# polimi-ispl/deep_prior_interpolation

Hardware: AMD Instinct MI355X
Metric: Adam iters/sec on 3D MultiRes-UNet (whole job over n_gpus; per_gpu beside it); recon SNR(dB) vs ref under config.snr_vs_reference (higher is better)
Workload: dtype f32

## Files before the change

### deep_prior_interpolation_amd/csrc/api.cpp

```cpp
#include <stdarg.h>
#include <string.h>
#include "common.h"

static thread_local char g_err[512] = "";

void dpi_set_error(const char* fmt, ...) {
  va_list ap;
  va_start(ap, fmt);
  vsnprintf(g_err, sizeof(g_err), fmt, ap);
  va_end(ap);
}

int dpi_check_launch(const char* what) {
  const hipError_t e = hipGetLastError();
  if (e != hipSuccess) {
    dpi_set_error("%s: %s", what, hipGetErrorString(e));
    return DPI_E_LAUNCH;
  }
  return DPI_OK;
}

extern "C" const char* dpi_last_error(void) { return g_err; }
extern "C" int dpi_version(void) { return 406; }
extern "C" int dpi_conv_desc_size(void) { return (int)sizeof(dpi_conv_desc); }

extern "C" int dpi_device_info(int device, int* cus, int* lds_bytes, size_t* hbm_bytes, char* name, int name_len) {
  hipDeviceProp_t p;
  const hipError_t e = hipGetDeviceProperties(&p, device);
  if (e != hipSuccess) {
    dpi_set_error("device_info: %s", hipGetErrorString(e));
    return DPI_E_LAUNCH;
  }
  if (cus) *cus = p.multiProcessorCount;
  if (lds_bytes) *lds_bytes = (int)p.sharedMemPerBlock;
  if (hbm_bytes) *hbm_bytes = p.totalGlobalMem;
  if (name && name_len > 0) {
    strncpy(name, p.gcnArchName, name_len - 1);
    name[name_len - 1] = 0;
  }
  return DPI_OK;
}

__global__ void dpi_marker_kernel() {}

extern "C" int dpi_profile_marker(int id, void* stream) {
  DPI_REQUIRE(id >= 1 && id < 65536, "profile_marker: id %d out of range", id);
  dpi_marker_kernel<<<(unsigned)id, 64, 0, (hipStream_t)stream>>>();
  return dpi_check_launch("profile_marker");
}

extern "C" int dpi_set_option(const char* key, int value) {
  DPI_REQUIRE(key != nullptr, "set_option: key is NULL");
  struct Entry { const char* key; int lo, hi; void (*set)(int); };
  static const Entry table[] = {
      {"splitk", 0, 1, dpi_set_splitk},
      {"dual_bwd_data", 0, 1, dpi_set_dual_bwd_data},
      {"bw_pair", 0, 2, dpi_set_bw_pair},
      {"bw_workgroups", 1, 1 << 24, [](int v) { dpi_set_bw_tuning(v, -1); }},
      {"bw_xcd_order", 0, 1, [](int v) { dpi_set_bw_tuning(0, v); }},
      {"mfma_min_cout", 0, 1 << 20, dpi_set_mfma_min_cout},
      {"bwd_weight_mfma_min_cout", 0, 1 << 20, dpi_set_bwd_weight_mfma_min_cout},
      {"fewco_mfma", 0, 1, dpi_set_fewco_mfma},
      {"q4", 0, 2, [](int v) { dpi_set_q4(v, -1); }},
      {"q4_ck", 0, 4, [](int v) { dpi_set_q4(-1, v); }},
      {"q4_debug", 0, 0xFFFF, dpi_set_q4_debug},
      {"bf16_debug", 0, 0x7F, dpi_set_bf16_debug},
  };
  for (const Entry& e : table)
    if (strcmp(key, e.key) == 0) {
      DPI_REQUIRE(value >= e.lo && value <= e.hi && !(strcmp(key, "q4_ck") == 0 && value != 0 && value != 2 && value != 4),
                  "set_option: %s = %d out of range [%d, %d]", key, value, e.lo, e.hi);
      e.set(value);
      return DPI_OK;
    }
  dpi_set_error("set_option: unknown key '%s'", key);
  return DPI_E_ARG;
}
```

### deep_prior_interpolation_amd/csrc/conv_mfma.hip

```cpp
#include "common.h"

void dpi_conv_out_dims(const dpi_conv_desc* d, int* Do, int* Ho, int* Wo);

namespace {

typedef float f32x4 __attribute__((ext_vector_type(4)));

struct MArgs {
  const float* __restrict__ x;
  const float* __restrict__ chain;
  const float* __restrict__ w;
  const float* __restrict__ bias;
  float* __restrict__ y;
  double* __restrict__ partials;
  int Cin, Cout;
  int D, H, W;
  int ntd, nth, ntw;
  long w_out_stride, w_in_stride;
  int accumulate;
  int split_cps;
  const float* __restrict__ x2;
  const float* __restrict__ w2;
  int C2;
  long w2_co_stride, w2_c_stride;
  int xb, yb;
  int ny;
};

template <int KD, int NR, int NH, int S = 1>
struct Geo {
  static constexpr bool SLICES = (KD == 3 && NR >= 4);
  static constexpr int SD = KD == 3 ? S : 1;
  static constexpr int TZ = SLICES ? 4 : 1;
  static constexpr int TY = SLICES ? NR : 4 * NR;
  static constexpr int TW = 16 * NH;
  static constexpr int ID = (TZ - 1) * SD + KD;
  static constexpr int IH = (TY - 1) * S + 3;
  static constexpr int IW = (TW - 1) * S + 3;
  static constexpr int RS = (IW + 3) & ~3;
  static constexpr int DS0 = IH * RS;
  static constexpr int DS = (S == 1 && (RS % 32) == 4) ? DS0 + ((12 - (DS0 % 32)) + 32) % 32 : DS0;
  static constexpr int CS0 = ID * DS;
  static constexpr int CSM = S == 1 ? 16 : 1;
  static constexpr int CS = CS0 + ((CSM - (CS0 % 32)) + 32) % 32;
  static constexpr int TILE = ID * IH * IW;
  static constexpr int E = (TILE + 255) / 256;
  static constexpr int NROW = (NR - 1) * S + 3;
  static constexpr int NSTEP = KD * NROW;
  static constexpr int NB = 3 * NH;
};

__device__ __forceinline__ int xcd_tile(int bid, int ntiles) {
  const int q = ntiles >> 3, r = ntiles & 7, xcd = bid & 7, i = bid >> 3;
  return (xcd < r ? xcd * (q + 1) : r * (q + 1) + (xcd - r) * q) + i;
}

template <class G>
__device__ __forceinline__ void tile_slots(int tid, int id0, int ih0, int iw0, int D, int H, int W, int (&goff)[G::E], int (&loff)[G::E]) {
#pragma unroll
  for (int e = 0; e < G::E; ++e) {
    const int idx = tid + e * 256;
    const int col = idx % G::IW, row = idx / G::IW;
    const int hy = row % G::IH, dz = row / G::IH;
    const int gd = id0 + dz, gh = ih0 + hy, gw = iw0 + col;
    const bool ok = idx < G::TILE && gd >= 0 && gd < D && gh >= 0 && gh < H && gw >= 0 && gw < W;
    goff[e] = ok ? (gd * H + gh) * W + gw : -1;
    loff[e] = idx < G::TILE ? dz * G::DS + hy * G::RS + col : -1;
  }
}

template <class G>
__device__ __forceinline__ void stage_load(float (&sr)[4][G::E], const float* __restrict__ x, int Cin, size_t V, int c0,
                                           const int (&goff)[G::E], bool xb = false) {
  if (xb) {
#pragma unroll
    for (int c = 0; c < 4; ++c) {
      const int ci = min(c0 + c, Cin - 1);
      const __amdgpu_buffer_rsrc_t r = dpi_buffer_t(dpi_at(x, (size_t)ci * V, true), V, true);
#pragma unroll
      for (int e = 0; e < G::E; ++e) sr[c][e] = dpi_buffer_load_bf16_raw(r, goff[e]);
    }
    return;
  }
#pragma unroll
  for (int c = 0; c < 4; ++c) {
    const int ci = min(c0 + c, Cin - 1);
    const __amdgpu_buffer_rsrc_t r = dpi_buffer(x + (size_t)ci * V, V * sizeof(float));
#pragma unroll
    for (int e = 0; e < G::E; ++e) sr[c][e] = dpi_buffer_load(r, goff[e] * 4);
  }
}

template <class G>
__device__ __forceinline__ void stage_store(float* lds, const float (&sr_in)[4][G::E], const float* __restrict__ chain, int Cin, int c0,
                                            const int (&goff)[G::E], const int (&loff)[G::E], bool xb = false) {
  float sr[4][G::E];
#pragma unroll
  for (int c = 0; c < 4; ++c)
#pragma unroll
    for (int e = 0; e < G::E; ++e) sr[c][e] = sr_in[c][e];
  if (xb) {
#pragma unroll
    for (int c = 0; c < 4; ++c)
#pragma unroll
      for (int e = 0; e < G::E; ++e) sr[c][e] = dpi_widen_raw(sr[c][e]);
  }
  if (chain == nullptr) {
#pragma unroll
    for (int c = 0; c < 4; ++c)
#pragma unroll
      for (int e = 0; e < G::E; ++e)
        if ((e + 1) * 256 <= G::TILE || loff[e] >= 0) lds[c * G::CS + loff[e]] = sr[c][e];
    return;
  }
#pragma unroll
  for (int c = 0; c < 4; ++c) {
    const int ci = min(c0 + c, Cin - 1);
    const Chain t = load_chain(chain, ci);
#pragma unroll
    for (int e = 0; e < G::E; ++e) {
      const float v = goff[e] >= 0 ? apply_chain(t, sr[c][e]) : sr[c][e];
      if ((e + 1) * 256 <= G::TILE || loff[e] >= 0) lds[c * G::CS + loff[e]] = v;
    }
  }
}

template <int KD, int NR, int NH>
struct GeoV2 {
  static constexpr int TY = 4 * NR, TW = 16 * NH;
  static constexpr int ID = KD == 3 ? 3 : 1, IH = (TY - 1) * 2 + 3;
  static constexpr int NQ = TW / 2 + 1;
  static constexpr int PW = 2 * NQ;
  static constexpr int RS = 2 * PW;
  static constexpr int DS = IH * RS;
  static constexpr int CS0 = ID * DS;
  static constexpr int CS = CS0 + ((16 - (CS0 % 32)) + 32) % 32;
  static constexpr int NV4 = ID * IH * NQ;
  static constexpr int E = (NV4 + 255) / 256;
};
template <class GV>
__device__ __forceinline__ void tile_slots_v(int tid, int id0, int ih0, int iw0, int D, int H, int W, int (&goff)[GV::E], int (&loff)[GV::E]) {
#pragma unroll
  for (int e = 0; e < GV::E; ++e) {
    const int idx = tid + e * 256;
    const int q = idx % GV::NQ, row = idx / GV::NQ;
    const int hy = row % GV::IH, dz = row / GV::IH;
    const int gd = id0 + dz, gh = ih0 + hy, gw = iw0 + 4 * q;
    const bool ok = idx < GV::NV4 && gd >= 0 && gd < D && gh >= 0 && gh < H && gw >= 0 && gw + 4 <= W;
    goff[e] = ok ? (gd * H + gh) * W + gw : -4;
    loff[e] = idx < GV::NV4 ? dz * GV::DS + hy * GV::RS + 2 * q : -1;
  }
}
template <class GV>
// ... 877 lines not shown
      for (int t = 0; t < TAPS; ++t) wr[t] = ok ? wn[t] : 0.f;
    }
    __syncthreads();
#pragma unroll
    for (int c = 0; c < 4; ++c)
#pragma unroll
      for (int e = 0; e < E; ++e)
        if ((e + 1) * 256 <= TILE || loff[e] >= 0) lds[c * CS + loff[e]] = a.dyb ? dpi_widen_raw(sr[c][e]) : sr[c][e];
    __syncthreads();
    if (c0 + 4 < a.Cout) fetch(c0 + 4);
#pragma unroll
    for (int sd = 0; sd < ID; ++sd)
#pragma unroll
      for (int ir = 0; ir < 3; ++ir)
#pragma unroll
        for (int sw = 0; sw < 2; ++sw) {
          const float b = lds[lbase + (sd * IH + ir) * RS + sw];
#pragma unroll
          for (int sh = 0; sh < 2; ++sh) {
            const int row = ir - sh;
            if (row < 0 || row > 1) continue;
#pragma unroll
            for (int cls = 0; cls < NCLS; ++cls) {
              const int pw = cls & 1, ph = (cls >> 1) & 1, pd = KD == 3 ? (cls >> 2) & 1 : 0;
              if ((sw && !pw) || (sh && !ph) || (sd && !pd)) continue;
              const int kw = pw ? (sw ? 0 : 2) : 1, kh = ph ? (sh ? 0 : 2) : 1, kd = KD == 3 ? (pd ? (sd ? 0 : 2) : 1) : 0;
              acc[cls][row] = __builtin_amdgcn_mfma_f32_16x16x4f32(wr[(kd * 3 + kh) * 3 + kw], b, acc[cls][row], 0, 0, 0);
            }
          }
        }
  }
  typedef float f32x2 __attribute__((ext_vector_type(2)));
  const bool vec2 = !a.dxb && ((a.W | (int)(V & 1)) & 1) == 0 && (((uintptr_t)a.dx) & 7) == 0;
  if (vec2) {
#pragma unroll
    for (int cp = 0; cp < NCLS / 2; ++cp) {
      const int ph = cp & 1, pd = KD == 3 ? (cp >> 1) & 1 : 0;
#pragma unroll
      for (int row = 0; row < 2; ++row) {
        const int id = KD == 3 ? 2 * md0 + pd : md0, ih = 2 * (mh0 + wid * 2 + row) + ph, iw = 2 * (mw0 + lj);
        if (id < a.D && ih < a.H && iw < a.W) {
          f32x2 old[4];
#pragma unroll
          for (int r = 0; r < 4; ++r) {
            const int ci = n0 + 4 * lk + r;
            const size_t o = (size_t)min(ci, a.Cin - 1) * V + ((size_t)id * a.H + ih) * a.W + iw;
            old[r] = a.accumulate ? *reinterpret_cast<const f32x2*>(a.dx + o) : (f32x2){0.f, 0.f};
          }
#pragma unroll
          for (int r = 0; r < 4; ++r) {
            const int ci = n0 + 4 * lk + r;
            if (ci < a.Cin) {
              const size_t o = (size_t)ci * V + ((size_t)id * a.H + ih) * a.W + iw;
              const f32x2 v = a.accumulate ? (f32x2){old[r][0] + acc[2 * cp][row][r], old[r][1] + acc[2 * cp + 1][row][r]}
                                           : (f32x2){acc[2 * cp][row][r], acc[2 * cp + 1][row][r]};
              *reinterpret_cast<f32x2*>(a.dx + o) = v;
            }
          }
        }
      }
    }
    return;
  }
#pragma unroll
  for (int cls = 0; cls < NCLS; ++cls) {
    const int pw = cls & 1, ph = (cls >> 1) & 1, pd = KD == 3 ? (cls >> 2) & 1 : 0;
#pragma unroll
    for (int row = 0; row < 2; ++row) {
      const int id = KD == 3 ? 2 * md0 + pd : md0, ih = 2 * (mh0 + wid * 2 + row) + ph, iw = 2 * (mw0 + lj) + pw;
      if (id < a.D && ih < a.H && iw < a.W) {
#pragma unroll
        for (int r = 0; r < 4; ++r) {
          const int ci = n0 + 4 * lk + r;
          if (ci < a.Cin) {
            const size_t o = (size_t)ci * V + ((size_t)id * a.H + ih) * a.W + iw;
            dpi_st(a.dx, o, a.accumulate ? dpi_ld(a.dx, o, a.dxb) + acc[cls][row][r] : acc[cls][row][r], a.dxb);
          }
        }
      }
    }
  }
}

__global__ __launch_bounds__(256) void splitk_reduce_kernel(const float* __restrict__ ws, int nsplit, const float* __restrict__ bias,
                                                            float* __restrict__ y, int accumulate, double* __restrict__ partials,
                                                            int Cout, size_t Vo, size_t per, bool yb) {
  const int lane = threadIdx.x & 63, co = blockIdx.y * 4 + (threadIdx.x >> 6);
  if (co >= Cout) return;
  const size_t lo = (size_t)blockIdx.x * per, hi = lo + per < Vo ? lo + per : Vo;
  const float bv = bias ? bias[co] : 0.f;
  double sum = 0.0, sq = 0.0;
  for (size_t v = lo + lane; v < hi; v += 64) {
    float t = ws[(size_t)co * Vo + v];
    for (int sp = 1; sp < nsplit; ++sp) t += ws[((size_t)sp * Cout + co) * Vo + v];
    t += bv;
    if (accumulate) t += dpi_ld(y, (size_t)co * Vo + v, yb);
    t = dpi_stored(t, yb);
    dpi_st(y, (size_t)co * Vo + v, t, yb);
    sum += t; sq += (double)t * t;
  }
  if (partials) {
#pragma unroll
    for (int o = 32; o > 0; o >>= 1) { sum += __shfl_xor(sum, o, 64); sq += __shfl_xor(sq, o, 64); }
    if (lane == 0) { partials[((size_t)blockIdx.x * Cout + co) * 2] = sum; partials[((size_t)blockIdx.x * Cout + co) * 2 + 1] = sq; }
  }
}

}

void dpi_mfma_variant(const dpi_conv_desc* d, int cout, int* nr, int* nh) {
  int Do, Ho, Wo;
  dpi_conv_out_dims(d, &Do, &Ho, &Wo);
  const int tz = d->kd == 3 ? 4 : 1, ty = d->kd == 3 ? 8 : 32;
  const long nb = (long)cdiv(Do, tz) * cdiv(Ho, ty) * cdiv(Wo, 32) * cdiv(cout, 16);
  if (nb >= 512 && d->stride == 1) { *nr = 8; *nh = 2; }
  else { *nr = 2; *nh = Wo > 16 ? 2 : 1; }
}

bool dpi_mfma_half_tile(const dpi_conv_desc* d, bool flip) {
  const int cin = flip ? d->Cout : d->Cin, cout = flip ? d->Cin : d->Cout;
  int nr, nh;
  dpi_mfma_variant(d, cout, &nr, &nh);
  if (nr != 8 || d->kd != 3) return false;
  if (cin == 1) return true;
  if (cin <= 8) return false;
  return flip || ((cin & 3) == 1);
}

int dpi_mfma_tiles(const dpi_conv_desc* d, int nr, int nh, int* ntd, int* nth, int* ntw) {
  int Do, Ho, Wo;
  dpi_conv_out_dims(d, &Do, &Ho, &Wo);
  const bool slices = d->kd == 3 && nr >= 4;
  const int tz = slices ? 4 : 1, ty = slices ? nr : 4 * nr;
  *ntd = cdiv(Do, tz); *nth = cdiv(Ho, ty); *ntw = cdiv(Wo, 16 * nh);
  return *ntd * *nth * *ntw;
}

template <int KD, bool FLIP, bool IOB = false>
static void launch_variant(const MArgs& a_in, int nr, int nh, int stride, dim3 grid_in, hipStream_t st) {
  if constexpr (!IOB) {
    if (a_in.xb || a_in.yb) { launch_variant<KD, FLIP, true>(a_in, nr, nh, stride, grid_in, st); return; }
  }
  const bool persistent = stride == 1 && nr == 8 && a_in.Cin > 8;
  MArgs a = a_in;
  dim3 grid = grid_in;
  if (!persistent && grid_in.y > 1) {
    a.ny = (int)grid_in.y;
    grid = dim3(8 * ((grid_in.x + 7) / 8) * grid_in.y, 1, grid_in.z);
  }
  if (stride == 2) {
    if constexpr (!FLIP) {
      if constexpr (!IOB) {
        static const bool s2v = getenv("DPI_NO_S2V") == nullptr;
        if (s2v && a.W % 4 == 0 && (((size_t)a.D * a.H * a.W) & 3) == 0 && ((uintptr_t)a.x & 15) == 0) {
          if (nh == 2) conv_mfma_kernel<KD, 2, 2, false, 2, 2, false, false, false, false, true><<<grid, 256, 0, st>>>(a);
          else conv_mfma_kernel<KD, 2, 1, false, 2, 2, false, false, false, false, true><<<grid, 256, 0, st>>>(a);
          return;
        }
      }
      if (nh == 2) conv_mfma_kernel<KD, 2, 2, false, 2, 2, false, false, IOB><<<grid, 256, 0, st>>>(a);
      else conv_mfma_kernel<KD, 2, 1, false, 2, 2, false, false, IOB><<<grid, 256, 0, st>>>(a);
    }
    return;
  }
  const bool tailpack = (a.Cin & 3) == 1 && (a.Cin > 4 || a.Cin == 1);
  if (nr == 4) {
    if constexpr (KD == 3) {
      if (tailpack) conv_mfma_kernel<KD, 4, 2, FLIP, 1, 3, false, true, IOB><<<grid, 256, 0, st>>>(a);
      else conv_mfma_kernel<KD, 4, 2, FLIP, 1, 3, false, false, IOB><<<grid, 256, 0, st>>>(a);
    }
    return;
  }
  if (nr == 8) {
    static const bool persist = getenv("DPI_NO_PERSIST") == nullptr;
    dim3 pg = grid;
    static const bool yloop = getenv("DPI_YLOOP") != nullptr && getenv("DPI_YLOOP")[0] == '1';
    if constexpr (KD == 3 && FLIP && !IOB) {
      if (yloop && a.Cin <= 4 && a.ny > 1 && a.split_cps == 0 && grid_in.z == 1) {
        conv_mfma_kernel<KD, 8, 2, FLIP, 1, 2, false, false, IOB, true><<<dim3(8 * ((grid_in.x + 7) / 8), 1, 1), 256, 0, st>>>(a);
        return;
      }
    }
    if (a.Cin <= 8) conv_mfma_kernel<KD, 8, 2, FLIP, 1, 3, false, false, IOB><<<grid, 256, 0, st>>>(a);
    else {
      if (persist && grid.x > 512) pg.x = 512;
      if (tailpack) conv_mfma_kernel<KD, 8, 2, FLIP, 1, 2, true, true, IOB><<<pg, 256, 0, st>>>(a);
      else conv_mfma_kernel<KD, 8, 2, FLIP, 1, 2, true, false, IOB><<<pg, 256, 0, st>>>(a);
    }
  }
  else if (nh == 2) conv_mfma_kernel<KD, 2, 2, FLIP, 1, 2, false, false, IOB><<<grid, 256, 0, st>>>(a);
  else conv_mfma_kernel<KD, 2, 1, FLIP, 1, 2, false, false, IOB><<<grid, 256, 0, st>>>(a);
}

#ifdef DPI_TRACE
extern "C" int dpi_debug_read_blocks(long long* out) { return (int)hipMemcpyFromSymbol(out, HIP_SYMBOL(g_blk), sizeof(long long) * 8192 * 4); }
extern "C" int dpi_debug_read_trace(long long* out) { return (int)hipMemcpyFromSymbol(out, HIP_SYMBOL(g_trace), sizeof(long long) * 4 * 64); }
#endif
static int g_splitk = getenv("DPI_SPLITK") ? atoi(getenv("DPI_SPLITK")) : 1;
extern "C" void dpi_set_splitk(int on) { g_splitk = on; }
int dpi_mfma_splitk(const dpi_conv_desc* d, bool flip) {
  if (!g_splitk || d->k != 3) return 1;
  const int cin = flip ? d->Cout : d->Cin, cout = flip ? d->Cin : d->Cout;
  int nr, nh, a, b, c;
  dpi_mfma_variant(d, cout, &nr, &nh);
  if (nr != 2 || dpi_mfma_half_tile(d, flip)) return 1;
  const long wgs = (long)dpi_mfma_tiles(d, nr, nh, &a, &b, &c) * cdiv(cout, 16);
  const int chunks = cdiv(cin, 4);
  if (wgs > 512 || (wgs > 256 && chunks < 24)) return 1;
  long ns = 1536 / wgs;
  if (ns > chunks / 8) ns = chunks / 8;
  if (ns > 8) ns = 8;
  return ns < 2 ? 1 : (int)ns;
}
size_t dpi_conv_mfma_ws_floats(const dpi_conv_desc* d, bool flip) {
  const int ns = dpi_mfma_splitk(d, flip);
  if (ns < 2) return 0;
  int Do, Ho, Wo;
  dpi_conv_out_dims(d, &Do, &Ho, &Wo);
  return (size_t)ns * (flip ? d->Cin : d->Cout) * Do * Ho * Wo;
}

bool dpi_conv_mfma_second_ok(const dpi_conv_desc* d, bool flip, int C2, bool have_ws) {
  int Do, Ho, Wo;
  dpi_conv_out_dims(d, &Do, &Ho, &Wo);
  if (!flip || d->stride != 1 || C2 < 1 || ((size_t)C2 + 4) * Do * Ho * Wo * sizeof(float) >= ((size_t)1 << 31)) return false;
  int nr, nh;
  dpi_mfma_variant(d, d->Cin, &nr, &nh);
  if (nr == 8 && !dpi_mfma_half_tile(d, flip) && d->Cout > 8) return false;
  return !(have_ws && dpi_mfma_splitk(d, flip) > 1);
}

int dpi_conv_mfma_run(const dpi_conv_desc* d, const float* x, const float* chain, const float* w, const float* bias, float* y,
                      double* partials, bool flip, int accumulate, float* ws, size_t ws_floats, hipStream_t st, const MfmaSecond* sec) {
  const int taps = d->kd * 9;
  const int cin = flip ? d->Cout : d->Cin, cout = flip ? d->Cin : d->Cout;
  const long w_out = flip ? taps : (long)d->Cin * taps, w_in = flip ? (long)d->Cin * taps : taps;
  MArgs a{x, chain, w, bias, y, partials, cin, cout, d->D, d->H, d->W, 0, 0, 0, w_out, w_in, accumulate, 0, nullptr, nullptr, 0, 0, 0,
          dpi_io_in(d, flip), dpi_io_out(d, flip)};
  int nr, nh;
  dpi_mfma_variant(d, cout, &nr, &nh);
  if (dpi_mfma_half_tile(d, flip)) nr = 4;
  const int ntiles = dpi_mfma_tiles(d, nr, nh, &a.ntd, &a.nth, &a.ntw);
  dim3 grid(ntiles, cdiv(cout, 16));
  if (sec) { a.x2 = sec->x2; a.w2 = sec->w2; a.C2 = sec->C2; a.w2_co_stride = sec->w2_co_stride; a.w2_c_stride = sec->w2_c_stride; }
  const int nsplit = (ws && !sec) ? dpi_mfma_splitk(d, flip) : 1;
  if (nsplit > 1) {
    int Do, Ho, Wo;
    dpi_conv_out_dims(d, &Do, &Ho, &Wo);
    const size_t Vo = (size_t)Do * Ho * Wo;
    DPI_REQUIRE(ws_floats >= (size_t)nsplit * cout * Vo, "conv (split): workspace of %zu floats, need %zu", ws_floats, (size_t)nsplit * cout * Vo);
    a.split_cps = 4 * cdiv(cdiv(cin, 4), nsplit);
    a.y = ws; a.bias = nullptr; a.partials = nullptr; a.accumulate = 0; a.yb = 0;
    grid.z = cdiv(cin, a.split_cps);
    const int nz = (int)grid.z;
    if (d->kd == 3) { if (flip) launch_variant<3, true>(a, nr, nh, d->stride, grid, st); else launch_variant<3, false>(a, nr, nh, d->stride, grid, st); }
    else { if (flip) launch_variant<1, true>(a, nr, nh, d->stride, grid, st); else launch_variant<1, false>(a, nr, nh, d->stride, grid, st); }
    if (int e = dpi_check_launch("conv_mfma (split)")) return e;
    splitk_reduce_kernel<<<dim3(ntiles, cdiv(cout, 4)), 256, 0, st>>>(ws, nz, bias, y, accumulate, partials, cout, Vo, cdivz(Vo, (size_t)ntiles),
                                                                      dpi_io_out(d, flip));
    return dpi_check_launch("splitk_reduce");
  }
  if (d->kd == 3) { if (flip) launch_variant<3, true>(a, nr, nh, d->stride, grid, st); else launch_variant<3, false>(a, nr, nh, d->stride, grid, st); }
  else { if (flip) launch_variant<1, true>(a, nr, nh, d->stride, grid, st); else launch_variant<1, false>(a, nr, nh, d->stride, grid, st); }
  return dpi_check_launch("conv_mfma");
}

static bool mfma_bw_swap_better(const dpi_conv_desc* d) {
  if (d->stride != 1) return false;
  auto util = [](int rows, int staged) { return (double)rows / (16.0 * cdiv(rows, 16)) * staged / (4.0 * cdiv(staged, 4)); };
  return util(d->Cin, d->Cout) > 1.15 * util(d->Cout, d->Cin);
}

static int g_bw_want = getenv("DPI_BW_WANT") ? atoi(getenv("DPI_BW_WANT")) : 2304;
static int g_bw_xcd_order = getenv("DPI_BW_XCD_ORDER") ? atoi(getenv("DPI_BW_XCD_ORDER")) : 0;
extern "C" void dpi_set_bw_tuning(int want_workgroups, int xcd_order) {
  if (want_workgroups > 0) g_bw_want = want_workgroups;
  if (xcd_order >= 0) g_bw_xcd_order = xcd_order;
}
static size_t bw_extra_lds() { static const size_t v = getenv("DPI_BW_EXTRA_LDS") ? (size_t)atoi(getenv("DPI_BW_EXTRA_LDS")) * 1024 : 0; return v; }
struct MfmaBwPlan { int nchunks, tiles_per_chunk, ntiles, ntd, nth, ntw, nr, nh, npairs, nfull, ny; };
static int g_bw_pair = getenv("DPI_BW_PAIR") ? atoi(getenv("DPI_BW_PAIR")) : 2;
extern "C" void dpi_set_bw_pair(int mode) { if (mode >= 0 && mode <= 2) g_bw_pair = mode; }
static MfmaBwPlan mfma_bw_plan(const dpi_conv_desc* d, bool swap = false) {
  MfmaBwPlan p{};
  {
    const int staged = swap ? d->Cout : d->Cin, groups = cdiv(staged, 4);
    const bool s1k3 = d->stride == 1 && d->kd == 3;
    const int tailg = (s1k3 && (staged & 3) == 1) ? 1 : 0;
    p.nfull = groups - tailg;
    p.npairs = (g_bw_pair && s1k3 && !g_bw_xcd_order && p.nfull >= 2 && d->io == 0) ? p.nfull / 2 : 0;
    if (g_bw_pair == 2) {
      int a_, b_, c_;
      if (p.nfull < 4 || dpi_mfma_tiles(d, 8, 2, &a_, &b_, &c_) < 1024) p.npairs = 0;
    }
    p.ny = p.npairs ? p.npairs + (p.nfull & 1) + tailg : groups;
  }
  if (d->stride == 1) { p.nr = 8; p.nh = 2; }
  else { int Do, Ho, Wo; dpi_conv_out_dims(d, &Do, &Ho, &Wo); p.nr = 2; p.nh = Wo > 16 ? 2 : 1; }
  p.ntiles = dpi_mfma_tiles(d, p.nr, p.nh, &p.ntd, &p.nth, &p.ntw);
  const size_t per = (size_t)d->Cout * d->Cin * d->kd * 9;
  const size_t max_chunks_mem = per ? ((size_t)32 << 20) / per : 1;
  const size_t blocks_other = (size_t)p.ny * (swap ? cdiv(d->Cin, 16) : cdiv(d->Cout, 16));
  size_t want = (size_t)g_bw_want / blocks_other;
  if (want < 1) want = 1;
  if (want > (size_t)p.ntiles) want = p.ntiles;
  if (want > max_chunks_mem) want = max_chunks_mem;
// ... 134 lines not shown
```

### deep_prior_interpolation_amd/csrc/dpi_hip_internal.h

```cpp
#pragma once
#define DPI_INTERNAL __attribute__((visibility("hidden")))
extern "C" {
DPI_INTERNAL void dpi_set_bw_tuning(int want_workgroups, int xcd_order);
DPI_INTERNAL void dpi_set_bf16_debug(int flags);
DPI_INTERNAL void dpi_set_splitk(int on);
DPI_INTERNAL void dpi_set_dual_bwd_data(int on);
DPI_INTERNAL void dpi_set_bw_pair(int mode);
DPI_INTERNAL void dpi_set_mfma_min_cout(int n);
DPI_INTERNAL void dpi_set_bwd_weight_mfma_min_cout(int n);
DPI_INTERNAL void dpi_set_fewco_mfma(int on);
DPI_INTERNAL void dpi_set_q4(int on, int ck);
DPI_INTERNAL void dpi_set_q4_debug(int flags);
}
```

Before: 33.97.

## Add dedicated stride-2 forward MFMA conv kernel with multi-Cout-tile register reuse

Adds a new stride-2 3x3x3 forward conv kernel that deinterleaves even and odd input columns into LDS, keeps all 27 weight taps in registers, and computes two 16-wide output-channel groups per block (MT=2). This reuses each staged input tile across more output channels and prefetches the next channel chunk's input and weights while the current one computes. It is enabled by default when the layer has at least two Cout groups. The cost is higher register pressure and a new code path that duplicates the epilogue and stats-partials logic.

```diff
diff --git a/deep_prior_interpolation_amd/csrc/api.cpp b/deep_prior_interpolation_amd/csrc/api.cpp
--- a/deep_prior_interpolation_amd/csrc/api.cpp
+++ b/deep_prior_interpolation_amd/csrc/api.cpp
@@ -65,6 +65,7 @@
       {"q4_ck", 0, 4, [](int v) { dpi_set_q4(-1, v); }},
       {"q4_debug", 0, 0xFFFF, dpi_set_q4_debug},
       {"bf16_debug", 0, 0x7F, dpi_set_bf16_debug},
+      {"s2_fwd", 0, 2, dpi_set_s2_fwd},
   };
   for (const Entry& e : table)
     if (strcmp(key, e.key) == 0) {
diff --git a/deep_prior_interpolation_amd/csrc/conv_mfma.hip b/deep_prior_interpolation_amd/csrc/conv_mfma.hip
--- a/deep_prior_interpolation_amd/csrc/conv_mfma.hip
+++ b/deep_prior_interpolation_amd/csrc/conv_mfma.hip
@@ -1,4 +1,5 @@
 #include "common.h"
+#include "conv_s2_mfma.h"
 
 void dpi_conv_out_dims(const dpi_conv_desc* d, int* Do, int* Ho, int* Wo);
 
@@ -1182,6 +1183,14 @@
     if constexpr (!FLIP) {
       if constexpr (!IOB) {
         static const bool s2v = getenv("DPI_NO_S2V") == nullptr;
+        if constexpr (KD == 3) {
+          const S2FwdArgs f{a.x, a.chain, a.w, a.bias, a.y, a.partials, a.Cin, a.Cout, a.D, a.H, a.W, a.ntd, a.nth, a.ntw,
+                            a.w_out_stride, a.w_in_stride, a.accumulate, a.split_cps, (int)grid_in.y};
+          if (a.x2 == nullptr && dpi_conv_s2_fwd_wanted(f)) {
+            dpi_conv_s2_fwd_launch(f, nh, (int)grid_in.x, (int)grid_in.z, st);
+            return;
+          }
+        }
         if (s2v && a.W % 4 == 0 && (((size_t)a.D * a.H * a.W) & 3) == 0 && ((uintptr_t)a.x & 15) == 0) {
           if (nh == 2) conv_mfma_kernel<KD, 2, 2, false, 2, 2, false, false, false, false, true><<<grid, 256, 0, st>>>(a);
           else conv_mfma_kernel<KD, 2, 1, false, 2, 2, false, false, false, false, true><<<grid, 256, 0, st>>>(a);
diff --git a/deep_prior_interpolation_amd/csrc/conv_s2_mfma.h b/deep_prior_interpolation_amd/csrc/conv_s2_mfma.h
--- /dev/null
+++ b/deep_prior_interpolation_amd/csrc/conv_s2_mfma.h
@@ -0,0 +1,23 @@
+#pragma once
+#include <hip/hip_runtime.h>
+
+struct S2FwdArgs {
+  const float* x;
+  const float* chain;
+  const float* w;
+  const float* bias;
+  float* y;
+  double* partials;
+  int Cin, Cout;
+  int D, H, W;
+  int ntd, nth, ntw;
+  long w_out_stride, w_in_stride;
+  int accumulate;
+  int split_cps;
+  int ny;
+};
+
+int dpi_s2_fwd_mode();
+bool dpi_conv_s2_fwd_can(const S2FwdArgs& a);
+bool dpi_conv_s2_fwd_wanted(const S2FwdArgs& a);
+void dpi_conv_s2_fwd_launch(const S2FwdArgs& a, int nh, int ntiles, int nz, hipStream_t st);
diff --git a/deep_prior_interpolation_amd/csrc/conv_s2_mfma.hip b/deep_prior_interpolation_amd/csrc/conv_s2_mfma.hip
--- /dev/null
+++ b/deep_prior_interpolation_amd/csrc/conv_s2_mfma.hip
@@ -0,0 +1,287 @@
+#include <stdlib.h>
+#include "common.h"
+#include "conv_s2_mfma.h"
+
+namespace {
+
+typedef float f32x4 __attribute__((ext_vector_type(4)));
+typedef float f32x2 __attribute__((ext_vector_type(2)));
+
+template <int NH>
+struct S2Geo {
+  static constexpr int NR = 2, TY = 4 * NR, TW = 16 * NH;
+  static constexpr int ID = 3, IH = (TY - 1) * 2 + 3;
+  static constexpr int NQ = TW / 2 + 1;
+  static constexpr int PW = 2 * NQ;
+  static constexpr int RS = 2 * PW;
+  static constexpr int DS = IH * RS;
+  static constexpr int CS0 = ID * DS;
+  static constexpr int CS = CS0 + ((16 - (CS0 % 32)) + 32) % 32;
+  static constexpr int NV4 = ID * IH * NQ;
+  static constexpr int E = (NV4 + 255) / 256;
+  static constexpr int NROW = (NR - 1) * 2 + 3;
+  static constexpr int NSTEP = ID * NROW;
+  static constexpr int NB = 3 * NH;
+};
+
+__device__ __forceinline__ int s2_xcd_tile(int bid, int ntiles) {
+  const int q = ntiles >> 3, r = ntiles & 7, xcd = bid & 7, i = bid >> 3;
+  return (xcd < r ? xcd * (q + 1) : r * (q + 1) + (xcd - r) * q) + i;
+}
+
+template <int NH, int MT>
+__global__ __launch_bounds__(256, 2) void conv_s2_fwd_mfma_kernel(S2FwdArgs a) {
+  using G = S2Geo<NH>;
+  constexpr int TAPS = 27, NR = G::NR, NT = NR * NH, E = G::E;
+  __shared__ __attribute__((aligned(16))) float lds[4 * G::CS];
+  __shared__ double red[4][16 * MT][2];
+
+  const int tid = threadIdx.x, lane = tid & 63, wid = tid >> 6;
+  const int lk = lane >> 4, lj = lane & 15;
+  const int ntiles = a.ntd * a.nth * a.ntw;
+  const int ngy = (a.ny + MT - 1) / MT;
+  int tile_id, yg;
+  {
+    const int q8 = ntiles >> 3, r8 = ntiles & 7, xcd = blockIdx.x & 7, j = blockIdx.x >> 3;
+    const int i = j / ngy;
+    yg = j - i * ngy;
+    if (i >= q8 + (xcd < r8 ? 1 : 0)) return;
+    tile_id = s2_xcd_tile(i * 8 + xcd, ntiles);
+  }
+  const int n0 = yg * 16 * MT;
+  const int nm = min(MT, a.ny - yg * MT);
+  const size_t V = (size_t)a.D * a.H * a.W;
+  const int Do = (a.D - 1) / 2 + 1, Ho = (a.H - 1) / 2 + 1, Wo = (a.W - 1) / 2 + 1;
+  const size_t Vo = (size_t)Do * Ho * Wo;
+  int od0, oh0, ow0;
+  {
+    int bt = tile_id;
+    const int tw_i = bt % a.ntw; bt /= a.ntw;
+    const int th_i = bt % a.nth; bt /= a.nth;
+    od0 = bt; oh0 = th_i * G::TY; ow0 = tw_i * G::TW;
+  }
+  const int wh = wid * NR;
+  const int lbase = lk * G::CS + wh * 2 * G::RS + lj;
+
+  int goff[E], loff[E];
+#pragma unroll
+  for (int e = 0; e < E; ++e) {
+    const int idx = tid + e * 256;
+    const int q = idx % G::NQ, row = idx / G::NQ;
+    const int hy = row % G::IH, dz = row / G::IH;
+    const int gd = 2 * od0 - 1 + dz, gh = 2 * oh0 - 1 + hy, gw = 2 * ow0 - 4 + 4 * q;
+    const bool ok = idx < G::NV4 && gd >= 0 && gd < a.D && gh >= 0 && gh < a.H && gw >= 0 && gw + 4 <= a.W;
+    goff[e] = ok ? (gd * a.H + gh) * a.W + gw : -4;
+    loff[e] = idx < G::NV4 ? dz * G::DS + hy * G::RS + 2 * q : -1;
+  }
+  f32x4 sv[4][E];
+  auto sload = [&](int c0) {
+#pragma unroll
+    for (int c = 0; c < 4; ++c) {
+      const int ci = min(c0 + c, a.Cin - 1);
+      const __amdgpu_buffer_rsrc_t r = dpi_buffer(a.x + (size_t)ci * V, V * sizeof(float));
+#pragma unroll
+      for (int e = 0; e < E; ++e) sv[c][e] = __builtin_bit_cast(f32x4, __builtin_amdgcn_raw_buffer_load_b128(r, goff[e] * 4, 0, 0));
+    }
+  };
+  auto sstore = [&](int c0) {
+    if (a.chain == nullptr) {
+#pragma unroll
+      for (int c = 0; c < 4; ++c)
+#pragma unroll
+        for (int e = 0; e < E; ++e)
+          if ((e + 1) * 256 <= G::NV4 || loff[e] >= 0) {
+            float* const p = lds + c * G::CS + loff[e];
+            *reinterpret_cast<f32x2*>(p) = (f32x2){sv[c][e][0], sv[c][e][2]};
+            *reinterpret_cast<f32x2*>(p + G::PW) = (f32x2){sv[c][e][1], sv[c][e][3]};
+          }
+      return;
+    }
+#pragma unroll
+    for (int c = 0; c < 4; ++c) {
+      const Chain t = load_chain(a.chain, min(c0 + c, a.Cin - 1));
+#pragma unroll
+      for (int e = 0; e < E; ++e) {
+        const float m = goff[e] >= 0 ? 1.f : 0.f;
+        if ((e + 1) * 256 <= G::NV4 || loff[e] >= 0) {
+          float* const p = lds + c * G::CS + loff[e];
+          *reinterpret_cast<f32x2*>(p) = (f32x2){m * apply_chain(t, sv[c][e][0]), m * apply_chain(t, sv[c][e][2])};
+          *reinterpret_cast<f32x2*>(p + G::PW) = (f32x2){m * apply_chain(t, sv[c][e][1]), m * apply_chain(t, sv[c][e][3])};
+        }
+      }
+    }
+  };
+
+  auto w_ptr = [&](int m, int c0, bool& ok) {
+    const int co = n0 + 16 * m + lj, ci = c0 + lk;
+    ok = co < a.Cout && ci < a.Cin;
+    return a.w + (ok ? co : 0) * a.w_out_stride + (ok ? ci : 0) * a.w_in_stride;
+  };
+  float wr[MT][TAPS], wn[MT][9];
+  auto load_w_raw = [&](int c0, int kd) {
+#pragma unroll
+    for (int m = 0; m < MT; ++m) {
+      bool ok;
+      const float* __restrict__ wp = w_ptr(m, c0, ok);
+#pragma unroll
+      for (int t = 0; t < 9; ++t) wn[m][t] = wp[kd * 9 + t];
+    }
+  };
+  auto commit_w = [&](int c0, int kd) {
+#pragma unroll
+    for (int m = 0; m < MT; ++m) {
+      const bool ok = n0 + 16 * m + lj < a.Cout && c0 + lk < a.Cin;
+#pragma unroll
+      for (int t = 0; t < 9; ++t) wr[m][kd * 9 + t] = ok ? wn[m][t] : 0.f;
+    }
+  };
+
+  const int c_lo = a.split_cps ? (int)blockIdx.z * a.split_cps : 0;
+  const int c_hi = a.split_cps ? min(c_lo + a.split_cps, a.Cin) : a.Cin;
+  float* __restrict__ const ybase = a.y + (size_t)blockIdx.z * a.Cout * Vo;
+  sload(c_lo);
+#pragma unroll
+  for (int m = 0; m < MT; ++m) {
+    bool ok;
+    const float* __restrict__ wp = w_ptr(m, c_lo, ok);
+#pragma unroll
+    for (int t = 0; t < TAPS; ++t) wr[m][t] = wp[t];
+#pragma unroll
+    for (int t = 0; t < TAPS; ++t) wr[m][t] = ok ? wr[m][t] : 0.f;
+  }
+
+  f32x4 acc[MT][NT];
+#pragma unroll
+  for (int m = 0; m < MT; ++m)
+#pragma unroll
+    for (int t = 0; t < NT; ++t) acc[m][t] = (f32x4){0.f, 0.f, 0.f, 0.f};
+  if (a.accumulate) {
+#pragma unroll
+    for (int m = 0; m < MT; ++m)
+#pragma unroll
+      for (int r = 0; r < 4; ++r) {
+        const int co = n0 + 16 * m + 4 * lk + r;
+#pragma unroll
+        for (int t = 0; t < NT; ++t) {
+          const int oh = oh0 + wh + t / NH, ow = ow0 + (t % NH) * 16 + lj;
+          if (co < a.Cout && oh < Ho && ow < Wo) acc[m][t][r] = ybase[(size_t)co * Vo + ((size_t)od0 * Ho + oh) * Wo + ow];
+        }
+      }
+  }
+
+  for (int c0 = c_lo; c0 < c_hi; c0 += 4) {
+    __syncthreads();
+    sstore(c0);
+    __syncthreads();
+    const bool more = c0 + 4 < c_hi;
+    if (more) sload(c0 + 4);
+    const int cn = more ? c0 + 4 : c_lo;
+    float bc[G::NB], bn[G::NB];
+    auto load_b = [&](float (&b)[G::NB], int step) {
+      const int kd = step / G::NROW, ir = step % G::NROW;
+#pragma unroll
+      for (int h = 0; h < NH; ++h)
+#pragma unroll
+        for (int kw = 0; kw < 3; ++kw)
+          b[h * 3 + kw] = lds[lbase + kd * G::DS + ir * G::RS + h * 16 + (kw == 1 ? 2 : G::PW + (kw == 0 ? 1 : 2))];
+    };
+    load_b(bc, 0);
+#pragma unroll
+    for (int step = 0; step < G::NSTEP; ++step) {
+      const int kd = step / G::NROW, ir = step % G::NROW;
+      if (step + 1 < G::NSTEP) load_b(bn, step + 1);
+      if (ir == 0) load_w_raw(cn, kd);
+      __builtin_amdgcn_sched_barrier(0);
+#pragma unroll
+      for (int m = 0; m < MT; ++m) {
+        if (m < nm) {
+#pragma unroll
+          for (int kw = 0; kw < 3; ++kw)
+#pragma unroll
+            for (int kh = 0; kh < 3; ++kh) {
+              const int hr = (ir - kh) / 2;
+              if (ir - kh >= 0 && (ir - kh) % 2 == 0 && hr < NR) {
+#pragma unroll
+                for (int h = 0; h < NH; ++h)
+                  acc[m][hr * NH + h] = __builtin_amdgcn_mfma_f32_16x16x4f32(wr[m][(kd * 3 + kh) * 3 + kw], bc[h * 3 + kw], acc[m][hr * NH + h], 0, 0, 0);
+              }
+            }
+        }
+      }
+      __builtin_amdgcn_sched_barrier(0);
+#pragma unroll
+      for (int i = 0; i < G::NB; ++i) bc[i] = bn[i];
+      if (ir == G::NROW - 1) commit_w(cn, kd);
+    }
+  }
+
+  const int vbase = (od0 * Ho + oh0 + wh) * Wo + ow0 + lj;
+#pragma unroll
+  for (int m = 0; m < MT; ++m) {
+    if (m >= nm) break;
+    const bool interior = oh0 + G::TY <= Ho && ow0 + G::TW <= Wo && n0 + 16 * m + 16 <= a.Cout;
+#pragma unroll
+    for (int r = 0; r < 4; ++r) {
+      const int co = n0 + 16 * m + 4 * lk + r;
+      const bool cok = co < a.Cout;
+      const float bv = (a.bias && cok) ? a.bias[co] : 0.f;
+      float* __restrict__ yc = ybase + (size_t)(cok ? co : 0) * Vo + vbase;
+      double s = 0.0, q = 0.0;
+      if (interior) {
+#pragma unroll
+        for (int t = 0; t < NT; ++t) {
+          const float v = acc[m][t][r] + bv;
+          yc[(t / NH) * Wo + (t % NH) * 16] = v;
+          if (a.partials) { s += v; q += (double)v * v; }
+        }
+      } else {
+#pragma unroll
+        for (int t = 0; t < NT; ++t) {
+          const int oh = oh0 + wh + t / NH, ow = ow0 + (t % NH) * 16 + lj;
+          if (cok && oh < Ho && ow < Wo) {
+            const float v = acc[m][t][r] + bv;
+            yc[(t / NH) * Wo + (t % NH) * 16] = v;
+            s += v;
+            q += (double)v * v;
+          }
+        }
+      }
+      if (a.partials) {
+#pragma unroll
+        for (int o = 8; o > 0; o >>= 1) { s += __shfl_xor(s, o, 64); q += __shfl_xor(q, o, 64); }
+        if (lj == 0) { red[wid][16 * m + 4 * lk + r][0] = s; red[wid][16 * m + 4 * lk + r][1] = q; }
+      }
+    }
+  }
+  if (a.partials) {
+    __syncthreads();
+    if (tid < 32 * nm) {
+      const int c = tid >> 1, which = tid & 1;
+      const double rsum = red[0][c][which] + red[1][c][which] + red[2][c][which] + red[3][c][which];
+      if (n0 + c < a.Cout) a.partials[((size_t)tile_id * a.Cout + n0 + c) * 2 + which] = rsum;
+    }
+  }
+}
+
+}
+
+static int g_s2_fwd = getenv("DPI_S2_FWD") ? atoi(getenv("DPI_S2_FWD")) : 1;
+extern "C" void dpi_set_s2_fwd(int mode) { g_s2_fwd = mode; }
+int dpi_s2_fwd_mode() { return g_s2_fwd; }
+
+bool dpi_conv_s2_fwd_can(const S2FwdArgs& a) {
+  return a.W % 4 == 0 && (((size_t)a.D * a.H * a.W) & 3) == 0 && ((uintptr_t)a.x & 15) == 0 && (size_t)a.D * a.H * a.W < ((size_t)1 << 29);
+}
+
+bool dpi_conv_s2_fwd_wanted(const S2FwdArgs& a) {
+  if (g_s2_fwd == 0 || !dpi_conv_s2_fwd_can(a)) return false;
+  if (g_s2_fwd == 2) return true;
+  return a.ny >= 2;
+}
+
+void dpi_conv_s2_fwd_launch(const S2FwdArgs& a, int nh, int ntiles, int nz, hipStream_t st) {
+  const int ngy = (a.ny + 1) / 2;
+  const dim3 grid(8 * ((ntiles + 7) / 8) * ngy, 1, nz);
+  if (nh == 2) conv_s2_fwd_mfma_kernel<2, 2><<<grid, 256, 0, st>>>(a);
+  else conv_s2_fwd_mfma_kernel<1, 2><<<grid, 256, 0, st>>>(a);
+}
diff --git a/deep_prior_interpolation_amd/csrc/dpi_hip_internal.h b/deep_prior_interpolation_amd/csrc/dpi_hip_internal.h
--- a/deep_prior_interpolation_amd/csrc/dpi_hip_internal.h
+++ b/deep_prior_interpolation_amd/csrc/dpi_hip_internal.h
@@ -11,4 +11,5 @@
 DPI_INTERNAL void dpi_set_fewco_mfma(int on);
 DPI_INTERNAL void dpi_set_q4(int on, int ck);
 DPI_INTERNAL void dpi_set_q4_debug(int flags);
+DPI_INTERNAL void dpi_set_s2_fwd(int mode);
 }
```

New measurement: 33.54, median of 2. 1.3% lower.
